# TUI-NICR/EMSANet

Hardware: AMD Instinct MI355X
Metric: images/sec (640x480 RGB-D, bs=32/GPU) fwd+bwd (higher is better)
Workload: dtype f32; 1 GPU; BASELINE.json configs[1]: full EMSANet RGB-D (resnet34-NBt1D x2, SE-add fusion, PPM, semantic+instance+orientation+scene heads), 640x480, bs=32/GPU, f32, train mode (BN batch stats, Dropout2d), step = fwd + bwd (fixed output cotangents) + grad all-reduce + SGD-nesterov update at lr 0 (fixed weights) replayed from a hipGraph; global_batch=32, parallelism=dp1, weights=random init (deterministic), mode=train-hipgraph

## Files before the change

emsanet_amd/_lib.py:

```python
import ctypes
import os
from ctypes import POINTER, Structure, c_char_p, c_float, c_int, c_int8, c_int32, c_int64, c_uint32, c_void_p

LIB_PATH = os.environ.get('EMSA_LIB') or os.path.join(
    os.path.dirname(os.path.abspath(__file__)), 'lib', 'libemsanet_hip.so')


class EmsaPackJob(Structure):
    _fields_ = [('src', c_void_p), ('dst0', c_void_p), ('dst1', c_void_p), ('cout', c_int32),
                ('cin', c_int32), ('kh', c_int32), ('kw', c_int32), ('kind', c_int32),
                ('first_block', c_int32), ('cout_total', c_int32), ('cout_off', c_int32),
                ('cin_total', c_int32), ('cin_off', c_int32)]


class EmsaDropoutJob(Structure):
    _fields_ = [('offset', c_int64), ('c', c_int32), ('layer_id', c_uint32), ('p', c_float),
                ('pad_', c_int32)]


class EmsaConvGeom(Structure):
    _fields_ = [
        ('n_img', c_int32),
        ('in_h', c_int32), ('in_w', c_int32),
        ('out_h', c_int32), ('out_w', c_int32),
# ... 27 lines not shown


_P = c_void_p
_GP = POINTER(EmsaConvGeom)
_TP = POINTER(EmsaTargetScale)

SIGNATURES = {
    'emsa_arch': (c_char_p, []),
    'emsa_version': (c_int, []),
    'emsa_set_batch_invariant': (c_int, [c_int]),
    'emsa_conv_igemm': (c_int, [_GP, _P, _P, _P, _P, _P, _P, _P, _P, c_int32, _P, c_int32, c_int32, _P]),
    'emsa_conv_stats_rows': (c_int, [_GP]),
    'emsa_conv1d_wino_supported': (c_int, [_GP]),
    'emsa_conv1d_wino_stats_rows': (c_int, [_GP]),
    'emsa_conv_relu_bits_words': (c_int64, [c_int64, c_int32]),
    'emsa_conv1d_wino_bnb': (c_int, [_GP, _P, _P, _P, _P, c_int32, _P, c_int32, _P, _P, _P, _P, _P,
                                     c_int32, _P]),
    'emsa_conv_igemm_bnb_t': (c_int, [c_int32, _GP, _P, _P, _P, _P, c_int32, _P, c_int32, _P, _P, _P, _P,
                                      _P, c_int32, _P]),
    'emsa_bn_bwd_apply_rows_t': (c_int, [c_int32, _P, _P, _P, _P, _P, _P, c_int32, c_int32, c_int64,
                                         c_int32, c_int32, _P, _P, _P, _P]),
    'emsa_conv1d_wino': (c_int, [_GP, _P, _P, _P, _P, _P, _P, _P, _P, c_int32, _P, c_int32, c_int32, _P,
                                 _P, _P]),
    'emsa_memset_async': (c_int, [_P, c_int32, c_int64, _P]),
    'emsa_graph_count_nodes': (c_int, [_P, POINTER(c_int32), POINTER(c_int32), POINTER(c_int32)]),
    'emsa_graph_replace_memsets': (c_int, [_P, POINTER(c_int32)]),
    'emsa_dropout2d_mask_batch': (c_int, [_P, _P, c_int32, c_int32, c_int32, c_uint32, _P, _P]),
    'emsa_to_nhwc_t': (c_int, [c_int32, _P, _P, c_int32, c_int32, c_int32, c_int32, c_int64, c_int64,
                               c_int64, c_int64, _P]),
    'emsa_conv1d_wino_resmask_supported': (c_int, [_GP, c_int32]),
    'emsa_conv1d_wino_resmask': (c_int, [_GP, _P, _P, _P, _P, c_int32, _P, _P]),
    'emsa_bn_act_fwd_wbits': (c_int, [_P, _P, _P, _P, _P, _P, c_int32, c_int64, c_int32, c_int32, _P, _P]),
    'emsa_bn_act_fwd_raff': (c_int, [_P] * 8 + [c_int32, c_int64, c_int32, c_int32, _P, c_int32, _P]),
    'emsa_bn_bwd_reduce_wbits': (c_int, [_P, _P, _P, _P, _P, _P, c_int32, c_int64, c_int32, _P, _P]),
    'emsa_bn_bwd_apply_wbits': (c_int, [_P] * 8 + [c_int32, c_int32, c_int64, c_int32, c_int32] + [_P] * 5),
    'emsa_conv1d_wino_inbn': (c_int, [_GP, _P, _P, _P, _P, _P, _P, _P, c_int32, _P, _P]),
    'emsa_conv_wgrad_inbn': (c_int, [_GP, _P, _P, _P, _P, _P, _P, _P, _P]),
    'emsa_conv_wgrad_inbn_t': (c_int, [c_int32, _GP, _P, _P, _P, _P, _P, _P, _P, _P]),
    'emsa_conv_wgrad_multi_inbn_t': (c_int, [c_int32, c_int32, _GP, POINTER(c_void_p), POINTER(c_void_p),
                                             POINTER(c_void_p), POINTER(c_void_p), _P,
                                             POINTER(c_void_p), POINTER(c_void_p), _P]),
    'emsa_conv1d_rs_inbn_t': (c_int, [c_int32, _GP, _P, _P, _P, _P, _P, _P, _P, c_int32, _P]),
    'emsa_bn_bwd_reduce_aff_t': (c_int, [c_int32, _P, _P, _P, _P, _P, _P, c_int32, c_int64, c_int32, _P, _P]),
    'emsa_bn_bwd_apply_aff_t': (c_int, [c_int32, _P, _P, _P, _P, _P, _P, _P, _P, c_int32, c_int32, c_int64,
                                        c_int32, _P, _P, _P, _P]),
    'emsa_conv_wgrad_multi_ws_bytes': (c_int64, [c_int32, c_int32, _GP]),
    'emsa_conv_wgrad_multi_t': (c_int, [c_int32, c_int32, _GP, POINTER(c_void_p), POINTER(c_void_p),
                                        POINTER(c_void_p), POINTER(c_void_p), _P, _P]),
    'emsa_pack_wino': (c_int, [_P, _P, _P, c_int32, c_int32, c_int32, _P]),
    'emsa_pack_batch': (c_int, [_P, c_int32, c_int32, _P]),
    'emsa_conv_wino2d_supported': (c_int, [_GP]),
    'emsa_conv_wino2d_stats_rows': (c_int, [_GP]),
    'emsa_conv_wino2d': (c_int, [_GP, _P, _P, _P, _P, _P, _P, _P, _P, c_int32, _P, c_int32, c_int32, _P]),
    'emsa_conv_wgrad_wino2d_supported': (c_int, [c_int32, _GP]),
    'emsa_conv_wgrad_wino2d_ws_bytes': (c_int64, [c_int32, _GP]),
    'emsa_conv_wgrad_wino2d_split_steps': (c_int, [c_int32, _GP]),
    'emsa_conv_wgrad_wino2d': (c_int, [c_int32, _GP, _P, _P, _P, _P, _P, c_int32, _P]),
    'emsa_pack_wino2d': (c_int, [_P, _P, _P, c_int32, c_int32, _P]),
    'emsa_pack_wino2d_packed': (c_int, [_P, _P, c_int32, c_int32, c_int32, _P]),
    'emsa_pack_wino_packed': (c_int, [_P, _P, c_int32, c_int32, c_int32, c_int32, _P]),
    'emsa_conv_wgrad_ws_bytes': (c_int64, [_GP]),
    'emsa_conv_wgrad': (c_int, [_GP, _P, _P, _P, _P, _P, _P]),
    'emsa_pack_weight_fwd': (c_int, [_P, _P] + [c_int32] * 8 + [_P]),
    'emsa_pack_weight_dgrad': (c_int, [_P, _P] + [c_int32] * 8 + [_P]),
    'emsa_unpack_wgrad': (c_int, [_P, _P] + [c_int32] * 8 + [_P]),
    'emsa_pack_weight_pair': (c_int, [_P, _P, _P] + [c_int32] * 4 + [_P]),
    'emsa_stem_pack_input': (c_int, [_P, _P, c_int32, c_int32, c_int32, c_int32, _P]),
    'emsa_stem_pack_weight': (c_int, [_P, _P, c_int32, c_int32, _P]),
    'emsa_stem_pack_input_rows_t': (c_int, [c_int32, _P, _P, c_int32, c_int32, c_int32, _P]),
    'emsa_stem_pack_weight_rows_t': (c_int, [c_int32, _P, _P, c_int32, _P]),
    'emsa_stem_unpack_wgrad_rows': (c_int, [_P, _P, c_int32, _P]),
    'emsa_stem_unpack_wgrad': (c_int, [_P, _P, c_int32, c_int32, _P]),
    'emsa_bn_finalize': (c_int, [_P, c_int32, c_int32, c_int64, _P, _P, c_float, c_float,
                                 _P, _P, _P, _P, _P, _P, _P, _P]),
    'emsa_bn_finalize_ws_bytes': (c_int, [c_int32]),
    'emsa_bn_fold': (c_int, [_P, _P, _P, _P, c_float, c_int32, _P, _P, _P, _P]),
    'emsa_relu_mask_words': (c_int64, [c_int64]),
    'emsa_bn_act_fwd': (c_int, [_P, _P, _P, _P, _P, _P, c_int32, c_int64, c_int32, c_int32, _P,
                                _P]),
    'emsa_bn_bwd_reduce': (c_int, [_P, _P, _P, _P, _P, _P, _P, c_int32, c_int64, c_int32, c_int32,
                                   _P, _P]),
    'emsa_bn_bwd_rows': (c_int, [c_int64, c_int32]),
    'emsa_bn_bwd_apply': (c_int, [_P, _P, _P, _P, _P, _P, _P, _P, _P, c_int32, c_int32, c_int64,
                                  c_int32, c_int32, c_int32, _P, _P, _P, _P, _P]),
    'emsa_dropout2d_mask': (c_int, [_P, c_int32, c_int32, c_float, c_uint32, c_uint32, _P]),
    'emsa_maxpool3x3s2_fwd': (c_int, [_P, _P, _P, c_int32, c_int32, c_int32, c_int32, _P]),
    'emsa_maxpool3x3s2_bwd': (c_int, [_P, _P, _P, c_int32, c_int32, c_int32, c_int32, _P]),
    'emsa_channel_ws_floats': (c_int, [c_int32, c_int64, c_int32]),
    'emsa_channel_mean': (c_int, [_P, _P, _P, c_int32, c_int64, c_int32, _P]),
    'emsa_se_mlp_fwd': (c_int, [_P] * 7 + [c_int32] * 3 + [_P]),
    'emsa_se_mlp_bwd': (c_int, [_P] * 11 + [c_int32] * 3 + [_P]),
    'emsa_se_scale_add_fwd': (c_int, [_P] * 5 + [c_int32, c_int64, c_int32, _P]),
    'emsa_se_scale_bwd_reduce': (c_int, [_P, _P, _P, _P, c_int32, c_int64, c_int32, _P]),
    'emsa_se_scale_bwd_apply': (c_int, [_P] * 5 + [c_int32, c_int64, c_int32, _P]),
    'emsa_up2x_dw3x3_fwd': (c_int, [_P] * 5 + [c_int32] * 4 + [_P]),
    'emsa_up2x_dw3x3_fwd_skipbn': (c_int, [_P] * 7 + [c_int32] * 4 + [_P]),
    'emsa_up2x_dw3x3_bwd_data': (c_int, [_P] * 3 + [c_int32] * 4 + [_P]),
    'emsa_up2x_dw3x3_bwd_weight': (c_int, [_P] * 4 + [c_int32] * 4 + [_P]),
    'emsa_up2x_dw3x3_bwd': (c_int, [_P] * 6 + [c_int32] * 4 + [_P]),
    'emsa_up2x_dw3x3_bwd_supported': (c_int, [c_int32, c_int32]),
    'emsa_adaptive_avgpool_fwd': (c_int, [_P, _P] + [c_int32] * 5 + [_P]),
    'emsa_adaptive_avgpool_bwd': (c_int, [_P, _P] + [c_int32] * 6 + [_P]),
    'emsa_bilinear_fwd': (c_int, [_P, _P] + [c_int32] * 7 + [_P]),
    'emsa_bilinear_bwd': (c_int, [_P, _P] + [c_int32] * 7 + [_P]),
    'emsa_head_act_fwd': (c_int, [_P, _P, c_int64] + [c_int32] * 5 + [_P]),
    'emsa_head_act_bwd': (c_int, [_P, _P, _P, _P, c_int64] + [c_int32] * 5 + [_P]),
# ... 185 lines not shown
```

emsanet_amd/csrc/conv_wino.hip:

```cpp
#include <cstdlib>

#include "common.h"
#include "prof.h"

namespace {

constexpr int kWK = 16;
constexpr int kWLD = kWK;
constexpr int kPairs = 32;

typedef unsigned int u32x4w __attribute__((ext_vector_type(4)));
typedef __bf16 wbf16x8 __attribute__((ext_vector_type(8)));
constexpr uint32_t kOOBw = 0x80000000u;
__device__ __forceinline__ __amdgpu_buffer_rsrc_t wrsrc(const void* p, uint32_t bytes) {
  return __builtin_amdgcn_make_buffer_rsrc(const_cast<void*>(p), 0, (int)bytes, 0x00020000);
}
__device__ __forceinline__ float4 wbuf_ld4(__amdgpu_buffer_rsrc_t r, uint32_t off) {
  return __builtin_bit_cast(float4, __builtin_amdgcn_raw_buffer_load_b128(r, (int)off, 0, 0));
}
__device__ __forceinline__ float4 wbuf_ld4s(__amdgpu_buffer_rsrc_t r, uint32_t voff, uint32_t soff) {
  return __builtin_bit_cast(float4,
                            __builtin_amdgcn_raw_buffer_load_b128(r, (int)voff, (int)soff, 0));
}
typedef float wf32x2 __attribute__((ext_vector_type(2)));
// ... 214 lines not shown
        acc[u] = __builtin_amdgcn_mfma_f32_32x32x2f32(v.z, fb[u].z, acc[u], 0, 0, 0);
#pragma unroll
      for (int u = 0; u < NT; ++u)
        acc[u] = __builtin_amdgcn_mfma_f32_32x32x2f32(v.w, fb[u].w, acc[u], 0, 0, 0);
    }
    }
#if EMSA_WINO_PRIO != 0
    __builtin_amdgcn_s_setprio(0);
#endif
    __syncthreads();
    if (has_next) store_lds(s + 1);
    __syncthreads();
  }

  constexpr int SLD = kWN + 4;
  constexpr int HP = kPairs / 2;
  constexpr uint32_t kNoPix = 0xFFFFFFFFu;
  float* const stage = smem;
  const int col4 = tid % NC4, n = n0 + col4 * 4;
  const int rgi = tid / NC4;
  const bool nok = n < p.n_ch;
  uint32_t lane_pix = kNoPix;
  {
    const int q = q0 + (lane >> 1);
    if (q < p.MP) {
      const int line = (int)wdiv((uint32_t)q, p.mul_pl, p.sh_pl);
      const int pp = q - line * p.PL;
      const int img = (int)wdiv((uint32_t)line, p.mul_a, p.sh_a);
      const int a = line - img * p.A;
      const int b = 2 * pp + (lane & 1);
      if (b < p.L) lane_pix = (uint32_t)(img * p.px_simg + a * p.px_sa + b * p.px_sb);
    }
  }
  wf32x2 ylo[PXI], yhi[PXI];
  uint32_t opix[PXI];
  bool ok[PXI];
  const float4 bv = (nok && p.bias) ? emsa_ld4(p.bias + n) : emsa_zero4();
  const wf32x2 blo = {bv.x, bv.y}, bhi = {bv.z, bv.w};
  const float sgo = (rgi & 1) ? -1.f : 1.f;
  const wf32x2 sg2o = {sgo, sgo};
  const int m03row = (rgi & 1) ? 3 : 0;
#pragma unroll
  for (int k = 0; k < PXI; ++k) {
    const uint32_t o = (uint32_t)__builtin_amdgcn_ds_bpermute((rgi + RG * k) * 4, (int)lane_pix);
    ok[k] = nok && o != kNoPix;
    opix[k] = o;
  }
  const __amdgpu_buffer_rsrc_t rs_out = wrsrc(p.out, kOOBw);
  const __amdgpu_buffer_rsrc_t rs_res = wrsrc(p.residual, kOOBw);
  const __amdgpu_buffer_rsrc_t rs_msk = wrsrc(p.mask_src, kOOBw);
  const __amdgpu_buffer_rsrc_t rs_mb = wrsrc(p.mask_bits, kOOBw);
  float4 rres[PXI], rmsk[PXI];
  wu32x2 rbits[PXI];
#pragma unroll
  for (int k = 0; k < PXI; ++k) {
    const bool live = ok[k];
    if (p.residual)
      rres[k] = wbuf_ld4(rs_res, live ? (opix[k] * (uint32_t)p.ld_res + (uint32_t)n) * 4u : kOOBw);
    if (p.mask_src)
      rmsk[k] = wbuf_ld4(rs_msk, live ? (opix[k] * (uint32_t)p.ld_mask + (uint32_t)n) * 4u : kOOBw);
    if constexpr (kWN == 64) {
      if (p.mask_bits)
        rbits[k] = __builtin_bit_cast(
            wu32x2, __builtin_amdgcn_raw_buffer_load_b64(
                        rs_mb, (int)(live ? (opix[k] * (uint32_t)p.tiles_n + (uint32_t)nt) * 8u
                                          : kOOBw), 0, 0));
    }
  }
#pragma unroll
  for (int h = 0; h < 2; ++h) {
  if (h) __syncthreads();
#pragma unroll
  for (int t = 0; t < NT; ++t)
#pragma unroll
    for (int r = 8 * h; r < 8 * h + 8; ++r) {
      const int row = (r & 3) + 8 * (r >> 2) + 4 * lh;
      stage[(wave * HP + row - HP * h) * SLD + t * 32 + l31] = acc[t][r];
    }
  __syncthreads();
#pragma unroll
  for (int k = h * (PXI / 2); k < (h + 1) * (PXI / 2); ++k) {
    const int px = rgi + RG * k;
    const int prl = (px >> 1) - HP * h;
    const float4 m1 = emsa_ld4(stage + (1 * HP + prl) * SLD + col4 * 4);
    const float4 m2 = emsa_ld4(stage + (2 * HP + prl) * SLD + col4 * 4);
    const float4 m03 = emsa_ld4(stage + (m03row * HP + prl) * SLD + col4 * 4);
    const wf32x2 tlo = wf32x2{m2.x, m2.y} + wf32x2{m03.x, m03.y};
    const wf32x2 thi = wf32x2{m2.z, m2.w} + wf32x2{m03.z, m03.w};
    ylo[k] = __builtin_elementwise_fma(tlo, sg2o, wf32x2{m1.x, m1.y}) + blo;
    yhi[k] = __builtin_elementwise_fma(thi, sg2o, wf32x2{m1.z, m1.w}) + bhi;
  }
  }

  if (p.stats != nullptr) {
    __syncthreads();
    float* red = smem;
    float* tmean = smem + RG * kWN;
    int* scnt = reinterpret_cast<int*>(tmean + kWN);
    wf32x2 s1lo = {0.f, 0.f}, s1hi = {0.f, 0.f};
    float wgt[PXI];
    int cnt = 0;
#pragma unroll
    for (int k = 0; k < PXI; ++k) {
      wgt[k] = ok[k] ? 1.f : 0.f;
      const wf32x2 w2 = {wgt[k], wgt[k]};
      s1lo = __builtin_elementwise_fma(ylo[k], w2, s1lo);
      s1hi = __builtin_elementwise_fma(yhi[k], w2, s1hi);
      cnt += ok[k] ? 1 : 0;
    }
    emsa_st4(red + rgi * kWN + col4 * 4, make_float4(s1lo.x, s1lo.y, s1hi.x, s1hi.y));
    if (col4 == 0) scnt[rgi] = cnt;
    __syncthreads();
    if (tid < kWN) {
      float a1 = 0.f;
#pragma unroll
      for (int g = 0; g < RG; ++g) a1 += red[g * kWN + tid];
      int c = 0;
#pragma unroll
      for (int g = 0; g < RG; ++g) c += scnt[g];
// ... 528 lines not shown
```

emsanet_amd/csrc/conv_wino2d.hip:

```cpp
#include "common.h"
#include "prof.h"

namespace {

constexpr int kK2 = 8;
constexpr int kTiles = 32;

typedef unsigned int u32x4v __attribute__((ext_vector_type(4)));
typedef float vf32x2 __attribute__((ext_vector_type(2)));
constexpr uint32_t kOOBw = 0x80000000u;
__device__ __forceinline__ __amdgpu_buffer_rsrc_t vrsrc(const void* p, uint32_t bytes) {
  return __builtin_amdgcn_make_buffer_rsrc(const_cast<void*>(p), 0, (int)bytes, 0x00020000);
}
__device__ __forceinline__ float4 vbuf_ld4(__amdgpu_buffer_rsrc_t r, uint32_t off) {
  return __builtin_bit_cast(float4, __builtin_amdgcn_raw_buffer_load_b128(r, (int)off, 0, 0));
}
__device__ __forceinline__ float4 vbuf_ld4s(__amdgpu_buffer_rsrc_t r, uint32_t voff, uint32_t soff) {
  return __builtin_bit_cast(float4,
                            __builtin_amdgcn_raw_buffer_load_b128(r, (int)voff, (int)soff, 0));
}
__device__ __forceinline__ uint32_t vdiv(uint32_t n, uint32_t mul, uint32_t sh) {
  return (__umulhi(n, mul) + n) >> sh;
}
__device__ __forceinline__ float4 sub4(float4 a, float4 b) {
  const vf32x2 lo = vf32x2{a.x, a.y} - vf32x2{b.x, b.y}, hi = vf32x2{a.z, a.w} - vf32x2{b.z, b.w};
  return make_float4(lo.x, lo.y, hi.x, hi.y);
}
__device__ __forceinline__ float4 add4(float4 a, float4 b) {
  const vf32x2 lo = vf32x2{a.x, a.y} + vf32x2{b.x, b.y}, hi = vf32x2{a.z, a.w} + vf32x2{b.z, b.w};
  return make_float4(lo.x, lo.y, hi.x, hi.y);
}

struct Wino2dArgs {
  const float* in;
  const float* u;
  float* out;
  const float* bias;
  float* stats;
  const float* scale;
  const float* shift;
  const float* residual;
  const float* mask_src;
  int ld_out, ld_res, ld_mask, act;
  int H, W, TH, TW, MT;
  int k_ch, n_ch;
  int in_simg, in_srow, in_spx;
  int tiles_m, tiles_n, ksteps;
  uint32_t in_bytes, u_bytes;
  uint32_t mul_tw, sh_tw, mul_th, sh_th;
};

template <int NT>
__global__ __launch_bounds__(256, NT == 1 ? 4 : 2) void conv_wino2d_kernel(const Wino2dArgs p) {
  constexpr int WN = 32 * NT;
  constexpr int NC4 = WN / 4;
  constexpr int RG = 256 / NC4;
  constexpr int PXH = 64 / RG;
  constexpr int PXI = 2 * PXH;
  constexpr int BLD = 16 * WN * 2 / 256;
  extern __shared__ __attribute__((aligned(16))) float smem[];
  float* const Hs = smem;
  float* const Us = smem + 16 * kTiles * kK2;

  const int tid = threadIdx.x, lane = tid & 63, wave = __builtin_amdgcn_readfirstlane(tid >> 6);
  const int l31 = lane & 31, lh = lane >> 5;
  const int wg = emsa_xcd_remap(blockIdx.x, gridDim.x);
  const int nt = wg % p.tiles_n, mt = wg / p.tiles_n;
  const int q0 = mt * kTiles, n0 = nt * WN;
  const __amdgpu_buffer_rsrc_t rs_in = vrsrc(p.in, p.in_bytes);
  const __amdgpu_buffer_rsrc_t rs_u = vrsrc(p.u, p.u_bytes);

  const int c4 = (tid & 1) * 4;
  const int ltile = (tid >> 1) & 31;
  uint32_t a_voff[4], b_voff[BLD];
  {
    const int q = q0 + ltile;
    int base = 0, y0 = 0;
    bool xok = false;
    if (q < p.MT) {
      const int line = (int)vdiv((uint32_t)q, p.mul_tw, p.sh_tw);
      const int tx = q - line * p.TW;
      const int img = (int)vdiv((uint32_t)line, p.mul_th, p.sh_th);
      const int ty = line - img * p.TH;
      const int x = 2 * tx - 1 + wave;
      y0 = 2 * ty;
      xok = x >= 0 && x < p.W;
      base = img * p.in_simg + y0 * p.in_srow + x * p.in_spx + c4;
    }
#pragma unroll
    for (int r = 0; r < 4; ++r) {
      const int y = y0 + r - 1;
      const bool ok = xok && y >= 0 && y < p.H;
      a_voff[r] = ok ? (uint32_t)(base + (r - 1) * p.in_srow) * 4u : kOOBw;
    }
  }
#pragma unroll
  for (int j = 0; j < BLD; ++j) {
    const int f = (tid >> 1) + 128 * j;
    const int comp = f / WN, n = n0 + (f % WN);
    b_voff[j] = n < p.n_ch ? (uint32_t)((comp * p.ksteps * p.n_ch + n) * kK2 + c4) * 4u : kOOBw;
  }
  const uint32_t last_oob = (p.ksteps - 1) * kK2 + c4 < p.k_ch ? 0u : kOOBw;
  float4 ra[4], rb[BLD];
  auto load_regs = [&](int s) {
    const uint32_t so = (uint32_t)(s * kK2) * 4u, sou = (uint32_t)(s * p.n_ch * kK2) * 4u;
    const uint32_t pm = (s + 1) * kK2 > p.k_ch ? 0xFFFFFFFFu : 0u;
#pragma unroll
    for (int r = 0; r < 4; ++r) ra[r] = vbuf_ld4s(rs_in, a_voff[r] | (last_oob & pm), so);
#pragma unroll
    for (int j = 0; j < BLD; ++j) rb[j] = vbuf_ld4s(rs_u, b_voff[j] | (last_oob & pm), sou);
  };
  auto store_lds = [&]() {
    float* const h = Hs + (wave * kTiles + ltile) * kK2 + c4;
    emsa_st4(h + 0 * 4 * kTiles * kK2, sub4(ra[0], ra[2]));
    emsa_st4(h + 1 * 4 * kTiles * kK2, add4(ra[1], ra[2]));
    emsa_st4(h + 2 * 4 * kTiles * kK2, sub4(ra[2], ra[1]));
    emsa_st4(h + 3 * 4 * kTiles * kK2, sub4(ra[1], ra[3]));
#pragma unroll
    for (int j = 0; j < BLD; ++j) emsa_st4(Us + ((tid >> 1) + 128 * j) * kK2 + c4, rb[j]);
  };

  const int ca = wave == 0 ? 0 : wave == 2 ? 2 : 1;
  const int cb = wave == 2 ? 1 : wave == 3 ? 3 : 2;
  const float sg = wave == 1 ? 1.f : -1.f;

  load_regs(0);
  f32x16 acc[4][NT];
#pragma unroll
  for (int i = 0; i < 4; ++i)
#pragma unroll
    for (int t = 0; t < NT; ++t)
#pragma unroll
      for (int r = 0; r < 16; ++r) acc[i][t][r] = 0.f;
  store_lds();
  __syncthreads();
  const float* const a0 = Hs + (ca * kTiles + l31) * kK2 + lh * 4;
  const float* const a1 = Hs + (cb * kTiles + l31) * kK2 + lh * 4;
  const float* const b = Us + (wave * WN + l31) * kK2 + lh * 4;
  for (int s = 0; s < p.ksteps; ++s) {
    const bool has_next = s + 1 < p.ksteps;
    __builtin_amdgcn_s_setprio(3);
    if (has_next) load_regs(s + 1);
    __builtin_amdgcn_s_setprio(1);
#pragma unroll
    for (int i = 0; i < 4; ++i) {
      const float4 x0 = emsa_ld4(a0 + i * 4 * kTiles * kK2), x1 = emsa_ld4(a1 + i * 4 * kTiles * kK2);
      const vf32x2 sg2 = {sg, sg};
      const vf32x2 vlo = __builtin_elementwise_fma(vf32x2{x1.x, x1.y}, sg2, vf32x2{x0.x, x0.y});
      const vf32x2 vhi = __builtin_elementwise_fma(vf32x2{x1.z, x1.w}, sg2, vf32x2{x0.z, x0.w});
      float4 fb[NT];
#pragma unroll
      for (int u = 0; u < NT; ++u) fb[u] = emsa_ld4(b + (i * 4 * WN + u * 32) * kK2);
#pragma unroll
      for (int u = 0; u < NT; ++u)
        acc[i][u] = __builtin_amdgcn_mfma_f32_32x32x2f32(vlo.x, fb[u].x, acc[i][u], 0, 0, 0);
#pragma unroll
      for (int u = 0; u < NT; ++u)
        acc[i][u] = __builtin_amdgcn_mfma_f32_32x32x2f32(vlo.y, fb[u].y, acc[i][u], 0, 0, 0);
#pragma unroll
      for (int u = 0; u < NT; ++u)
        acc[i][u] = __builtin_amdgcn_mfma_f32_32x32x2f32(vhi.x, fb[u].z, acc[i][u], 0, 0, 0);
#pragma unroll
      for (int u = 0; u < NT; ++u)
        acc[i][u] = __builtin_amdgcn_mfma_f32_32x32x2f32(vhi.y, fb[u].w, acc[i][u], 0, 0, 0);
    }
    __builtin_amdgcn_s_setprio(0);
    __syncthreads();
    if (has_next) store_lds();
    __syncthreads();
  }

  constexpr int SLD = WN + 4;
  constexpr uint32_t kNoPix = 0xFFFFFFFFu;
  float* const stage = smem;
  const int col4 = tid % NC4, n = n0 + col4 * 4;
  const int rgi = tid / NC4;
  const bool nok = n < p.n_ch;
  uint32_t lane_pix[2] = {kNoPix, kNoPix};
  {
    const int q = q0 + (lane >> 1);
    if (q < p.MT) {
      const int line = (int)vdiv((uint32_t)q, p.mul_tw, p.sh_tw);
      const int tx = q - line * p.TW;
      const int img = (int)vdiv((uint32_t)line, p.mul_th, p.sh_th);
      const int ty = line - img * p.TH;
      const int x = 2 * tx + (lane & 1);
#pragma unroll
      for (int a = 0; a < 2; ++a) {
        const int y = 2 * ty + a;
        if (x < p.W && y < p.H) lane_pix[a] = (uint32_t)((img * p.H + y) * p.W + x);
      }
    }
  }
  vf32x2 ylo[PXI], yhi[PXI];
  uint32_t opix[PXI];
  bool ok[PXI];
  const float4 bv = (nok && p.bias) ? emsa_ld4(p.bias + n) : emsa_zero4();
  const vf32x2 blo = {bv.x, bv.y}, bhi = {bv.z, bv.w};
  const float sgo = (rgi & 1) ? -1.f : 1.f;
  const vf32x2 sg2o = {sgo, sgo};
  const int m03row = (rgi & 1) ? 3 : 0;
#pragma unroll
  for (int k = 0; k < PXI; ++k) {
    const int a = k / PXH, kk = k % PXH;
    const uint32_t o = (uint32_t)__builtin_amdgcn_ds_bpermute((rgi + RG * kk) * 4, (int)lane_pix[a]);
    ok[k] = nok && o != kNoPix;
    opix[k] = o;
  }
  const __amdgpu_buffer_rsrc_t rs_out = vrsrc(p.out, kOOBw);
  const __amdgpu_buffer_rsrc_t rs_res = vrsrc(p.residual, kOOBw);
  const __amdgpu_buffer_rsrc_t rs_msk = vrsrc(p.mask_src, kOOBw);
  float4 rres[PXI], rmsk[PXI];
#pragma unroll
  for (int k = 0; k < PXI; ++k) {
    const bool live = ok[k];
    if (p.residual)
      rres[k] = vbuf_ld4(rs_res, live ? (opix[k] * (uint32_t)p.ld_res + (uint32_t)n) * 4u : kOOBw);
    if (p.mask_src)
      rmsk[k] = vbuf_ld4(rs_msk, live ? (opix[k] * (uint32_t)p.ld_mask + (uint32_t)n) * 4u : kOOBw);
  }
#pragma unroll
  for (int a = 0; a < 2; ++a) {
    __syncthreads();
#pragma unroll
    for (int t = 0; t < NT; ++t)
#pragma unroll
      for (int r = 0; r < 16; ++r) {
        const int row = (r & 3) + 8 * (r >> 2) + 4 * lh;
        const float v = a == 0 ? (acc[0][t][r] + acc[1][t][r]) + acc[2][t][r]
                               : (acc[1][t][r] - acc[2][t][r]) - acc[3][t][r];
        stage[(wave * kTiles + row) * SLD + t * 32 + l31] = v;
      }
    __syncthreads();
#pragma unroll
    for (int kk = 0; kk < PXH; ++kk) {
      const int k = a * PXH + kk;
      const int tl = (rgi + RG * kk) >> 1;
      const float4 m1 = emsa_ld4(stage + (1 * kTiles + tl) * SLD + col4 * 4);
      const float4 m2 = emsa_ld4(stage + (2 * kTiles + tl) * SLD + col4 * 4);
      const float4 m03 = emsa_ld4(stage + (m03row * kTiles + tl) * SLD + col4 * 4);
      const vf32x2 tlo = vf32x2{m2.x, m2.y} + vf32x2{m03.x, m03.y};
      const vf32x2 thi = vf32x2{m2.z, m2.w} + vf32x2{m03.z, m03.w};
      ylo[k] = __builtin_elementwise_fma(tlo, sg2o, vf32x2{m1.x, m1.y}) + blo;
      yhi[k] = __builtin_elementwise_fma(thi, sg2o, vf32x2{m1.z, m1.w}) + bhi;
    }
  }

  if (p.stats != nullptr) {
    __syncthreads();
    float* red = smem;
    float* tmean = smem + RG * WN;
    int* scnt = reinterpret_cast<int*>(tmean + WN);
    vf32x2 s1lo = {0.f, 0.f}, s1hi = {0.f, 0.f};
    float wgt[PXI];
    int cnt = 0;
#pragma unroll
    for (int k = 0; k < PXI; ++k) {
      wgt[k] = ok[k] ? 1.f : 0.f;
      const vf32x2 w2 = {wgt[k], wgt[k]};
      s1lo = __builtin_elementwise_fma(ylo[k], w2, s1lo);
      s1hi = __builtin_elementwise_fma(yhi[k], w2, s1hi);
      cnt += ok[k] ? 1 : 0;
    }
    emsa_st4(red + rgi * WN + col4 * 4, make_float4(s1lo.x, s1lo.y, s1hi.x, s1hi.y));
    if (col4 == 0) scnt[rgi] = cnt;
    __syncthreads();
    if (tid < WN) {
      float a1 = 0.f;
#pragma unroll
      for (int g = 0; g < RG; ++g) a1 += red[g * WN + tid];
      int c = 0;
#pragma unroll
// ... 50 lines not shown
      if (p.mask_src) {
        const float4 mm = rmsk[k];
        v.x = mm.x > 0.f ? v.x : 0.f; v.y = mm.y > 0.f ? v.y : 0.f;
        v.z = mm.z > 0.f ? v.z : 0.f; v.w = mm.w > 0.f ? v.w : 0.f;
      }
      if (p.act == EMSA_ACT_RELU) {
        v.x = fmaxf(v.x, 0.f); v.y = fmaxf(v.y, 0.f);
        v.z = fmaxf(v.z, 0.f); v.w = fmaxf(v.w, 0.f);
      }
      const uint32_t off = live ? (opix[k] * (uint32_t)p.ld_out + (uint32_t)n) * 4u : kOOBw;
      __builtin_amdgcn_raw_buffer_store_b128(__builtin_bit_cast(u32x4v, v), rs_out, (int)off, 0, 0);
    }
  }
}

__global__ void pack_wino2d_kernel(const float* __restrict__ w, float* __restrict__ u,
                                   float* __restrict__ ud, int cout, int cin) {
  const int total = cout * cin;
  for (int i = blockIdx.x * blockDim.x + threadIdx.x; i < total; i += gridDim.x * blockDim.x) {
    const int ci = i % cin, co = i / cin;
    float g[9], v[16];
#pragma unroll
    for (int t = 0; t < 9; ++t) g[t] = w[(size_t)i * 9 + t];
    emsa_wino2d_u(g, v);
#pragma unroll
    for (int c = 0; c < 16; ++c) {
      if (u) u[emsa_wino2d_at(c, co, ci, cout, cin)] = v[c];
      if (ud) ud[emsa_wino2d_at(emsa_wino2d_flip(c), ci, co, cin, cout)] = v[c];
    }
  }
}

__global__ void pack_wino2d_packed_kernel(const float* __restrict__ wp, float* __restrict__ u,
                                          int n, int k, int flip) {
  const int total = n * k;
  const size_t NK = (size_t)total;
  for (int i = blockIdx.x * blockDim.x + threadIdx.x; i < total; i += gridDim.x * blockDim.x) {
    float g[9], v[16];
#pragma unroll
    for (int t = 0; t < 9; ++t) g[t] = wp[(size_t)(flip ? 8 - t : t) * NK + i];
    emsa_wino2d_u(g, v);
#pragma unroll
    for (int c = 0; c < 16; ++c) u[emsa_wino2d_at(c, i / k, i % k, n, k)] = v[c];
  }
}

inline void magic2(uint32_t d, uint32_t& mul, uint32_t& sh) {
  uint32_t s = 0;
  while ((1ull << s) < d) ++s;
  sh = s;
  mul = (uint32_t)(((1ull << 32) * ((1ull << s) - d)) / d + 1);
}

}

extern "C" int emsa_pack_wino2d(const float* w_oihw, float* u, float* u_dgrad, int32_t cout,
                                int32_t cin, void* stream) {
  if (!w_oihw || (!u && !u_dgrad)) return EMSA_E_ARG;
  if (cout < 1 || cin < 1) return EMSA_E_SHAPE;
  int grid = (cout * cin + 255) / 256;
  if (grid > 2048) grid = 2048;
  hipLaunchKernelGGL(pack_wino2d_kernel, dim3(grid), dim3(256), 0, (hipStream_t)stream, w_oihw, u,
                     u_dgrad, cout, cin);
  return emsa_launch_status();
}

extern "C" int emsa_pack_wino2d_packed(const float* w_packed, float* u, int32_t n_ch, int32_t k_ch,
                                       int32_t flip, void* stream) {
  if (!w_packed || !u) return EMSA_E_ARG;
  if (n_ch < 1 || k_ch < 1) return EMSA_E_SHAPE;
  int grid = (n_ch * k_ch + 255) / 256;
  if (grid > 2048) grid = 2048;
  hipLaunchKernelGGL(pack_wino2d_packed_kernel, dim3(grid), dim3(256), 0, (hipStream_t)stream,
                     w_packed, u, n_ch, k_ch, flip ? 1 : 0);
  return emsa_launch_status();
}

extern "C" int emsa_conv_wino2d_supported(const EmsaConvGeom* g) {
  if (!g) return 0;
  if (g->out_pix_img || g->out_pix_row || g->out_pix_px || g->out_pix_off) return 0;
  auto tap3 = [](int off, int step) { return (off == -1 || off == 1) && step == -off; };
  if (!(g->kh == 3 && g->kw == 3 && tap3(g->off_w, g->step_w) && tap3(g->off_h, g->step_h) &&
        g->off_h == g->off_w))
    return 0;
  if (g->mul_h != 1 || g->mul_w != 1 || g->div_h != 1 || g->div_w != 1) return 0;
  if (g->n_img < 1 || g->in_h < 1 || g->in_w < 1 || g->k_ch < 4 || g->n_ch < 4) return 0;
  if (g->in_h != g->out_h || g->in_w != g->out_w) return 0;
  if ((g->k_ch & 3) || (g->n_ch & 3) || (g->ld_out & 3) || (g->in_px_stride & 3) ||
      (g->in_row_stride & 3) || (g->in_img_stride & 3))
    return 0;
  if ((long)g->n_img * g->in_img_stride >= (1L << 29)) return 0;
  if ((long)16 * g->n_ch * (g->k_ch + 7) >= (1L << 29)) return 0;
  return 1;
}

extern "C" int emsa_conv_wino2d_stats_rows(const EmsaConvGeom* g) {
  if (!emsa_conv_wino2d_supported(g)) return EMSA_E_SHAPE;
  const long mtl = (long)g->n_img * ((g->out_h + 1) / 2) * ((g->out_w + 1) / 2);
  return (int)((mtl + kTiles - 1) / kTiles);
}

extern "C" int emsa_conv_wino2d(const EmsaConvGeom* g, const float* in, const float* u2, float* out,
                                const float* bias, float* stats, const float* scale,
                                const float* shift, const float* residual, int32_t ld_res,
                                const float* mask_src, int32_t ld_mask, int32_t act,
                                void* stream) {
  if (!emsa_conv_wino2d_supported(g)) return EMSA_E_SHAPE;
  if (!in || !u2 || !out) return EMSA_E_ARG;
  if ((scale == nullptr) != (shift == nullptr)) return EMSA_E_ARG;
  if (stats && (scale || residual || mask_src || act != EMSA_ACT_NONE)) return EMSA_E_SHAPE;
  if (act != EMSA_ACT_NONE && act != EMSA_ACT_RELU) return EMSA_E_SHAPE;
  auto al16 = [](const void* q) { return (((uintptr_t)q) & 15) == 0; };
  if (!al16(in) || !al16(u2) || !al16(out) || !al16(bias) || !al16(scale) || !al16(shift) ||
      (residual && (!al16(residual) || (ld_res & 3))) ||
      (mask_src && (!al16(mask_src) || (ld_mask & 3))))
    return EMSA_E_SHAPE;
  Wino2dArgs a;
  a.in = in; a.u = u2; a.out = out; a.bias = bias; a.stats = stats; a.scale = scale;
  a.shift = shift; a.residual = residual; a.mask_src = mask_src;
  a.ld_out = g->ld_out; a.ld_res = ld_res; a.ld_mask = ld_mask; a.act = act;
  a.H = g->out_h; a.W = g->out_w;
  a.TH = (a.H + 1) / 2; a.TW = (a.W + 1) / 2;
  const long mtl = (long)g->n_img * a.TH * a.TW;
  {
    const long px = (long)g->n_img * a.H * a.W, lim = 1L << 29;
    if (px * g->ld_out >= lim || (residual && px * ld_res >= lim) ||
        (mask_src && px * ld_mask >= lim))
      return EMSA_E_SHAPE;
  }
  a.MT = (int)mtl;
  a.k_ch = g->k_ch; a.n_ch = g->n_ch;
  a.in_simg = (int)g->in_img_stride; a.in_srow = (int)g->in_row_stride; a.in_spx = g->in_px_stride;
  const int nt = g->n_ch % 64 == 0 ? 2 : 1;
  const int wn = 32 * nt;
  a.tiles_m = (a.MT + kTiles - 1) / kTiles;
  a.tiles_n = (g->n_ch + wn - 1) / wn;
  a.ksteps = (g->k_ch + kK2 - 1) / kK2;
  a.in_bytes = (uint32_t)((size_t)g->n_img * g->in_img_stride * sizeof(float));
  a.u_bytes = (uint32_t)((size_t)16 * a.ksteps * kK2 * g->n_ch * sizeof(float));
  magic2((uint32_t)a.TW, a.mul_tw, a.sh_tw);
  magic2((uint32_t)a.TH, a.mul_th, a.sh_th);
  const size_t lds_main = (size_t)(16 * kTiles + 16 * wn) * kK2 * sizeof(float);
  const size_t lds_epi = (size_t)4 * kTiles * (wn + 4) * sizeof(float);
  const size_t lds = lds_main > lds_epi ? lds_main : lds_epi;
  const double flops = 2.0 * g->n_img * a.H * a.W * (double)g->k_ch * g->n_ch * 9.0;
  const int ps = emsa_prof_begin(kProfClassWino3x3, flops, (hipStream_t)stream);
  if (nt == 2)
    hipLaunchKernelGGL((conv_wino2d_kernel<2>), dim3(a.tiles_m * a.tiles_n), dim3(256), lds,
                       (hipStream_t)stream, a);
  else
    hipLaunchKernelGGL((conv_wino2d_kernel<1>), dim3(a.tiles_m * a.tiles_n), dim3(256), lds,
                       (hipStream_t)stream, a);
  emsa_prof_end(ps, (hipStream_t)stream);
  return emsa_launch_status();
}
```

include/emsanet_hip.h:

```cpp
#ifndef EMSANET_HIP_H
#define EMSANET_HIP_H

#include <stdint.h>

#ifdef __cplusplus
extern "C" {
#endif

#define EMSA_OK 0
#define EMSA_E_SHAPE (-1)
#define EMSA_E_ARG (-2)
#define EMSA_E_LAUNCH (-3)

#define EMSA_ACT_NONE 0
#define EMSA_ACT_RELU 1

#define EMSA_DT_F32 0
#define EMSA_DT_BF16 1
#define EMSA_DT_F16 2

const char* emsa_arch(void);
int emsa_version(void);
int emsa_set_batch_invariant(int on);

// ... 4 lines not shown
  int32_t k_ch;
  int32_t n_ch;
  int32_t kh, kw;
  int32_t mul_h, off_h, step_h, div_h;
  int32_t mul_w, off_w, step_w, div_w;
  int64_t in_img_stride, in_row_stride;
  int32_t in_px_stride;
  int32_t ld_out;
  int32_t out_pix_img, out_pix_row, out_pix_px, out_pix_off;
} EmsaConvGeom;

int emsa_conv_igemm(const EmsaConvGeom* g, const float* in, const float* w, float* out,
                    const float* bias, float* stats, const float* scale, const float* shift,
                    const float* residual, int32_t ld_res, const float* mask_src,
                    int32_t ld_mask, int32_t act, void* stream);
int emsa_conv_stats_rows(const EmsaConvGeom* g);

int64_t emsa_conv_wgrad_ws_bytes(const EmsaConvGeom* g);
int emsa_conv_wgrad(const EmsaConvGeom* g, const float* in, const float* dout, float* dw,
                    float* dbias, float* ws, void* stream);

int emsa_conv1d_wino_supported(const EmsaConvGeom* g);
int emsa_conv1d_wino_stats_rows(const EmsaConvGeom* g);
int64_t emsa_conv_relu_bits_words(int64_t pixels, int32_t n_ch);
int emsa_conv1d_wino(const EmsaConvGeom* g, const float* in, const float* u, float* out,
                     const float* bias, float* stats, const float* scale, const float* shift,
                     const float* residual, int32_t ld_res, const float* mask_src,
                     int32_t ld_mask, int32_t act, const uint64_t* mask_bits,
                     uint64_t* relu_bits, void* stream);
int emsa_conv1d_wino_bnb(const EmsaConvGeom* g, const float* dy, const float* u, float* out,
                         const float* residual, int32_t ld_res, const float* t, int32_t ld_t,
                         const float* bn_scale, const float* bn_shift, const float* bn_mean,
                         const float* bn_invstd, float* partial, int32_t rows_alloc, void* stream);
int emsa_conv1d_wino_resmask_supported(const EmsaConvGeom* g, int32_t ld_res);
int emsa_conv1d_wino_resmask(const EmsaConvGeom* g, const float* dy, const float* u, float* out,
                             const float* residual, int32_t ld_res, const uint64_t* res_bits,
                             void* stream);
int emsa_conv1d_wino_inbn(const EmsaConvGeom* g, const float* in, const float* u, float* out,
                          const float* bias, float* stats, const float* in_scale,
                          const float* in_shift, int32_t act, uint64_t* relu_bits, void* stream);
int emsa_conv_wgrad_inbn(const EmsaConvGeom* g, const float* in, const float* dout, float* dw,
                         float* dbias, float* ws, const float* in_scale, const float* in_shift,
                         void* stream);
int emsa_pack_wino(const float* w_oihw, float* u, float* u_dgrad, int32_t cout, int32_t cin,
                   int32_t rows, void* stream);
int emsa_pack_wino_packed(const float* w_packed, float* u, int32_t n_ch, int32_t k_ch,
                          int32_t rows, int32_t flip, void* stream);
int emsa_conv_wino2d_supported(const EmsaConvGeom* g);
int emsa_conv_wino2d_stats_rows(const EmsaConvGeom* g);
int emsa_conv_wino2d(const EmsaConvGeom* g, const float* in, const float* u2, float* out,
                     const float* bias, float* stats, const float* scale, const float* shift,
                     const float* residual, int32_t ld_res, const float* mask_src,
                     int32_t ld_mask, int32_t act, void* stream);
int emsa_conv_wgrad_wino2d_supported(int32_t dtype, const EmsaConvGeom* g);
int64_t emsa_conv_wgrad_wino2d_ws_bytes(int32_t dtype, const EmsaConvGeom* g);
int emsa_conv_wgrad_wino2d_split_steps(int32_t dtype, const EmsaConvGeom* g);
int emsa_conv_wgrad_wino2d(int32_t dtype, const EmsaConvGeom* g, const void* in, const void* dout,
                           float* dw, float* dbias, float* ws, int32_t packed, void* stream);
int emsa_pack_wino2d(const float* w_oihw, float* u, float* u_dgrad, int32_t cout, int32_t cin,
                     void* stream);
int emsa_pack_wino2d_packed(const float* w_packed, float* u, int32_t n_ch, int32_t k_ch,
                            int32_t flip, void* stream);
typedef struct EmsaPackJob {
  const float* src;
  float* dst0;
  float* dst1;
  int32_t cout, cin, kh, kw;
  int32_t kind;
  int32_t first_block;
  int32_t cout_total, cout_off, cin_total, cin_off;
} EmsaPackJob;
int emsa_pack_batch(const EmsaPackJob* jobs_device, int32_t n_jobs, int32_t total_blocks,
                    void* stream);

int emsa_pack_weight_fwd(const float* w_oihw, float* w_packed, int32_t cout, int32_t cin,
                         int32_t kh, int32_t kw, int32_t cout_total, int32_t cout_off,
                         int32_t cin_total, int32_t cin_off,
                         void* stream);
int emsa_pack_weight_dgrad(const float* w_oihw, float* w_packed, int32_t cout, int32_t cin,
                           int32_t kh, int32_t kw, int32_t cout_total, int32_t cout_off,
                           int32_t cin_total, int32_t cin_off,
                           void* stream);
int emsa_pack_weight_pair(const float* w_oihw, float* w_packed_fwd, float* w_packed_dgrad,
                          int32_t cout, int32_t cin, int32_t kh, int32_t kw, void* stream);
int emsa_unpack_wgrad(const float* dw_packed, float* dw_oihw, int32_t cout, int32_t cin,
                      int32_t kh, int32_t kw, int32_t cout_total, int32_t cout_off,
                      int32_t cin_total, int32_t cin_off,
                      void* stream);

int emsa_stem_pack_input(const float* x_nchw, float* x_pad, int32_t n, int32_t c, int32_t h,
                         int32_t w, void* stream);
int emsa_stem_pack_weight(const float* w_oihw, float* w_packed, int32_t cout, int32_t cin,
                          void* stream);
int emsa_stem_unpack_wgrad(const float* dw_packed, float* dw_oihw, int32_t cout, int32_t cin,
                           void* stream);
int emsa_stem_pack_input_rows_t(int32_t dtype, const float* x, void* xp, int32_t n, int32_t h,
                                int32_t w, void* stream);
int emsa_stem_pack_weight_rows_t(int32_t dtype, const float* w, void* wp, int32_t cout, void* stream);
int emsa_stem_unpack_wgrad_rows(const float* dwp, float* dw, int32_t cout, void* stream);

int emsa_bn_finalize(const float* stats, int32_t rows, int32_t c, int64_t count,
                     const float* gamma, const float* beta, float eps, float momentum,
                     float* running_mean, float* running_var, float* scale, float* shift,
                     float* save_mean, float* save_invstd, void* ws, void* stream);
int emsa_bn_finalize_ws_bytes(int32_t c);
int emsa_bn_fold(const float* gamma, const float* beta, const float* running_mean,
// ... 526 lines not shown
```

Baseline: 345.6 images/s.

## Stage two K steps of input per barrier in 2D Winograd conv kernel

Adds a KS=16 variant of the 2D Winograd forward kernel. It loads and transforms input tiles for two K steps at once, so input loads and stores happen every other step with wider per-thread loads. By default it is used when NT=2 and k_ch>=40, and it can be overridden through an env var or a setter. It also splits the epilogue residual and mask loads into per-flag loops. In exchange it doubles the input LDS buffer, which lowers occupancy bounds, and it adds ablation macros for experiments.

```diff
diff --git a/emsanet_amd/_lib.py b/emsanet_amd/_lib.py
--- a/emsanet_amd/_lib.py
+++ b/emsanet_amd/_lib.py
@@ -103,6 +103,7 @@
     'emsa_conv_wino2d_supported': (c_int, [_GP]),
     'emsa_conv_wino2d_stats_rows': (c_int, [_GP]),
     'emsa_conv_wino2d': (c_int, [_GP, _P, _P, _P, _P, _P, _P, _P, _P, c_int32, _P, c_int32, c_int32, _P]),
+    'emsa_wino2d_set_stage': (c_int, [c_int]),
     'emsa_conv_wgrad_wino2d_supported': (c_int, [c_int32, _GP]),
     'emsa_conv_wgrad_wino2d_ws_bytes': (c_int64, [c_int32, _GP]),
     'emsa_conv_wgrad_wino2d_split_steps': (c_int, [c_int32, _GP]),
diff --git a/emsanet_amd/csrc/conv_wino.hip b/emsanet_amd/csrc/conv_wino.hip
--- a/emsanet_amd/csrc/conv_wino.hip
+++ b/emsanet_amd/csrc/conv_wino.hip
@@ -290,19 +290,26 @@
   const __amdgpu_buffer_rsrc_t rs_mb = wrsrc(p.mask_bits, kOOBw);
   float4 rres[PXI], rmsk[PXI];
   wu32x2 rbits[PXI];
-#pragma unroll
-  for (int k = 0; k < PXI; ++k) {
-    const bool live = ok[k];
-    if (p.residual)
-      rres[k] = wbuf_ld4(rs_res, live ? (opix[k] * (uint32_t)p.ld_res + (uint32_t)n) * 4u : kOOBw);
-    if (p.mask_src)
-      rmsk[k] = wbuf_ld4(rs_msk, live ? (opix[k] * (uint32_t)p.ld_mask + (uint32_t)n) * 4u : kOOBw);
-    if constexpr (kWN == 64) {
-      if (p.mask_bits)
+  if (p.residual) {
+#pragma unroll
+    for (int k = 0; k < PXI; ++k)
+      rres[k] =
+          wbuf_ld4(rs_res, ok[k] ? (opix[k] * (uint32_t)p.ld_res + (uint32_t)n) * 4u : kOOBw);
+  }
+  if (p.mask_src) {
+#pragma unroll
+    for (int k = 0; k < PXI; ++k)
+      rmsk[k] =
+          wbuf_ld4(rs_msk, ok[k] ? (opix[k] * (uint32_t)p.ld_mask + (uint32_t)n) * 4u : kOOBw);
+  }
+  if constexpr (kWN == 64) {
+    if (p.mask_bits) {
+#pragma unroll
+      for (int k = 0; k < PXI; ++k)
         rbits[k] = __builtin_bit_cast(
             wu32x2, __builtin_amdgcn_raw_buffer_load_b64(
-                        rs_mb, (int)(live ? (opix[k] * (uint32_t)p.tiles_n + (uint32_t)nt) * 8u
-                                          : kOOBw), 0, 0));
+                        rs_mb, (int)(ok[k] ? (opix[k] * (uint32_t)p.tiles_n + (uint32_t)nt) * 8u
+                                           : kOOBw), 0, 0));
     }
   }
 #pragma unroll
diff --git a/emsanet_amd/csrc/conv_wino2d.hip b/emsanet_amd/csrc/conv_wino2d.hip
--- a/emsanet_amd/csrc/conv_wino2d.hip
+++ b/emsanet_amd/csrc/conv_wino2d.hip
@@ -50,9 +50,17 @@
   uint32_t mul_tw, sh_tw, mul_th, sh_th;
 };
 
-template <int NT>
-__global__ __launch_bounds__(256, NT == 1 ? 4 : 2) void conv_wino2d_kernel(const Wino2dArgs p) {
+#ifndef EMSA_W2D_ABL
+#define EMSA_W2D_ABL 0
+#endif
+
+template <int NT, int KS>
+__global__ __launch_bounds__(256, NT == 2 ? 2 : KS == 16 ? 3 : 4) void conv_wino2d_kernel(
+    const Wino2dArgs p) {
+  static_assert(KS == 8 || KS == 16, "input stage of one or two K steps");
   constexpr int WN = 32 * NT;
+  constexpr int HSZ = 16 * kTiles * kK2;
+  constexpr int NA = KS / 2;
   constexpr int NC4 = WN / 4;
   constexpr int RG = 256 / NC4;
   constexpr int PXH = 64 / RG;
@@ -60,7 +68,7 @@
   constexpr int BLD = 16 * WN * 2 / 256;
   extern __shared__ __attribute__((aligned(16))) float smem[];
   float* const Hs = smem;
-  float* const Us = smem + 16 * kTiles * kK2;
+  float* const Us = smem + (KS / kK2) * HSZ;
 
   const int tid = threadIdx.x, lane = tid & 63, wave = __builtin_amdgcn_readfirstlane(tid >> 6);
   const int l31 = lane & 31, lh = lane >> 5;
@@ -70,61 +78,104 @@
   const __amdgpu_buffer_rsrc_t rs_in = vrsrc(p.in, p.in_bytes);
   const __amdgpu_buffer_rsrc_t rs_u = vrsrc(p.u, p.u_bytes);
 
-  const int c4 = (tid & 1) * 4;
-  const int ltile = (tid >> 1) & 31;
-  uint32_t a_voff[4], b_voff[BLD];
+  const int c4 = KS == 8 ? (tid & 1) * 4 : (tid & 3) * 4;
+  const int ltile = KS == 8 ? (tid >> 1) & 31 : (tid >> 2) & 31;
+  const int col0 = KS == 8 ? wave : 2 * (wave >> 1);
+  const int cu4 = (tid & 1) * 4;
+  constexpr int NBV = KS == 16 ? 1 : BLD;
+  uint32_t a_voff[NA], b_voff[NBV];
   {
     const int q = q0 + ltile;
-    int base = 0, y0 = 0;
-    bool xok = false;
+    int base = 0, y0 = 0, x0 = 0;
+    bool qok = false;
     if (q < p.MT) {
       const int line = (int)vdiv((uint32_t)q, p.mul_tw, p.sh_tw);
       const int tx = q - line * p.TW;
       const int img = (int)vdiv((uint32_t)line, p.mul_th, p.sh_th);
       const int ty = line - img * p.TH;
-      const int x = 2 * tx - 1 + wave;
+      x0 = 2 * tx - 1 + col0;
       y0 = 2 * ty;
-      xok = x >= 0 && x < p.W;
-      base = img * p.in_simg + y0 * p.in_srow + x * p.in_spx + c4;
-    }
-#pragma unroll
-    for (int r = 0; r < 4; ++r) {
-      const int y = y0 + r - 1;
-      const bool ok = xok && y >= 0 && y < p.H;
-      a_voff[r] = ok ? (uint32_t)(base + (r - 1) * p.in_srow) * 4u : kOOBw;
-    }
-  }
-#pragma unroll
-  for (int j = 0; j < BLD; ++j) {
+      qok = true;
+      base = img * p.in_simg + y0 * p.in_srow + x0 * p.in_spx + c4;
+    }
+#pragma unroll
+    for (int cc = 0; cc < NA / 4; ++cc) {
+      const int x = x0 + cc;
+      const bool xok = qok && x >= 0 && x < p.W;
+#pragma unroll
+      for (int r = 0; r < 4; ++r) {
+        const int y = y0 + r - 1;
+        const bool ok = xok && y >= 0 && y < p.H;
+        a_voff[cc * 4 + r] =
+            ok ? (uint32_t)(base + cc * p.in_spx + (r - 1) * p.in_srow) * 4u : kOOBw;
+#if EMSA_W2D_ABL & 1
+        a_voff[cc * 4 + r] = kOOBw;
+#endif
+      }
+    }
+  }
+#pragma unroll
+  for (int j = 0; j < NBV; ++j) {
     const int f = (tid >> 1) + 128 * j;
     const int comp = f / WN, n = n0 + (f % WN);
-    b_voff[j] = n < p.n_ch ? (uint32_t)((comp * p.ksteps * p.n_ch + n) * kK2 + c4) * 4u : kOOBw;
-  }
-  const uint32_t last_oob = (p.ksteps - 1) * kK2 + c4 < p.k_ch ? 0u : kOOBw;
-  float4 ra[4], rb[BLD];
-  auto load_regs = [&](int s) {
-    const uint32_t so = (uint32_t)(s * kK2) * 4u, sou = (uint32_t)(s * p.n_ch * kK2) * 4u;
-    const uint32_t pm = (s + 1) * kK2 > p.k_ch ? 0xFFFFFFFFu : 0u;
-#pragma unroll
-    for (int r = 0; r < 4; ++r) ra[r] = vbuf_ld4s(rs_in, a_voff[r] | (last_oob & pm), so);
-#pragma unroll
-    for (int j = 0; j < BLD; ++j) rb[j] = vbuf_ld4s(rs_u, b_voff[j] | (last_oob & pm), sou);
+    b_voff[j] = n < p.n_ch ? (uint32_t)((comp * p.ksteps * p.n_ch + n) * kK2 + cu4) * 4u : kOOBw;
+#if EMSA_W2D_ABL & 2
+    b_voff[j] = kOOBw;
+#endif
+  }
+  const int stages = (p.k_ch + KS - 1) / KS;
+  const uint32_t last_oob_a = (stages - 1) * KS + c4 < p.k_ch ? 0u : kOOBw;
+  const uint32_t last_oob_b = (p.ksteps - 1) * kK2 + cu4 < p.k_ch ? 0u : kOOBw;
+  const uint32_t b_jstride = (uint32_t)((128 / WN) * p.ksteps * p.n_ch * kK2) * 4u;
+  float4 ra[NA], rb[BLD];
+  auto load_a = [&](int S) {
+    const uint32_t so = (uint32_t)(S * KS) * 4u;
+    if constexpr (KS == 16) {
+      const uint32_t oob = c4 < p.k_ch - S * KS ? 0u : kOOBw;
+#pragma unroll
+      for (int r = 0; r < NA; ++r) ra[r] = vbuf_ld4s(rs_in, a_voff[r] | oob, so);
+    } else {
+      const uint32_t pm = (S + 1) * KS > p.k_ch ? 0xFFFFFFFFu : 0u;
+#pragma unroll
+      for (int r = 0; r < NA; ++r) ra[r] = vbuf_ld4s(rs_in, a_voff[r] | (last_oob_a & pm), so);
+    }
   };
-  auto store_lds = [&]() {
-    float* const h = Hs + (wave * kTiles + ltile) * kK2 + c4;
-    emsa_st4(h + 0 * 4 * kTiles * kK2, sub4(ra[0], ra[2]));
-    emsa_st4(h + 1 * 4 * kTiles * kK2, add4(ra[1], ra[2]));
-    emsa_st4(h + 2 * 4 * kTiles * kK2, sub4(ra[2], ra[1]));
-    emsa_st4(h + 3 * 4 * kTiles * kK2, sub4(ra[1], ra[3]));
-#pragma unroll
-    for (int j = 0; j < BLD; ++j) emsa_st4(Us + ((tid >> 1) + 128 * j) * kK2 + c4, rb[j]);
+  auto load_b = [&](int s) {
+    const uint32_t sou = (uint32_t)(s * p.n_ch * kK2) * 4u;
+    if constexpr (KS == 16) {
+      const uint32_t voff = b_voff[0] | (cu4 < p.k_ch - s * kK2 ? 0u : kOOBw);
+#pragma unroll
+      for (int j = 0; j < BLD; ++j) rb[j] = vbuf_ld4s(rs_u, voff, sou + (uint32_t)j * b_jstride);
+    } else {
+      const uint32_t pm = (s + 1) * kK2 > p.k_ch ? 0xFFFFFFFFu : 0u;
+#pragma unroll
+      for (int j = 0; j < BLD; ++j) rb[j] = vbuf_ld4s(rs_u, b_voff[j] | (last_oob_b & pm), sou);
+    }
+  };
+  auto store_a = [&]() {
+    float* const h = Hs + (KS == 16 && (tid & 2) ? HSZ : 0) + (col0 * kTiles + ltile) * kK2 +
+                     (tid & 1) * 4;
+#pragma unroll
+    for (int cc = 0; cc < NA / 4; ++cc) {
+      const float4* const d = ra + cc * 4;
+      float* const hc = h + cc * kTiles * kK2;
+      emsa_st4(hc + 0 * 4 * kTiles * kK2, sub4(d[0], d[2]));
+      emsa_st4(hc + 1 * 4 * kTiles * kK2, add4(d[1], d[2]));
+      emsa_st4(hc + 2 * 4 * kTiles * kK2, sub4(d[2], d[1]));
+      emsa_st4(hc + 3 * 4 * kTiles * kK2, sub4(d[1], d[3]));
+    }
+  };
+  auto store_b = [&]() {
+#pragma unroll
+    for (int j = 0; j < BLD; ++j) emsa_st4(Us + ((tid >> 1) + 128 * j) * kK2 + cu4, rb[j]);
   };
 
   const int ca = wave == 0 ? 0 : wave == 2 ? 2 : 1;
   const int cb = wave == 2 ? 1 : wave == 3 ? 3 : 2;
   const float sg = wave == 1 ? 1.f : -1.f;
 
-  load_regs(0);
+  load_a(0);
+  load_b(0);
   f32x16 acc[4][NT];
 #pragma unroll
   for (int i = 0; i < 4; ++i)
@@ -132,19 +183,17 @@
     for (int t = 0; t < NT; ++t)
 #pragma unroll
       for (int r = 0; r < 16; ++r) acc[i][t][r] = 0.f;
-  store_lds();
+  store_a();
+  store_b();
   __syncthreads();
   const float* const a0 = Hs + (ca * kTiles + l31) * kK2 + lh * 4;
   const float* const a1 = Hs + (cb * kTiles + l31) * kK2 + lh * 4;
   const float* const b = Us + (wave * WN + l31) * kK2 + lh * 4;
-  for (int s = 0; s < p.ksteps; ++s) {
-    const bool has_next = s + 1 < p.ksteps;
-    __builtin_amdgcn_s_setprio(3);
-    if (has_next) load_regs(s + 1);
-    __builtin_amdgcn_s_setprio(1);
+  auto mma = [&](int half) {
 #pragma unroll
     for (int i = 0; i < 4; ++i) {
-      const float4 x0 = emsa_ld4(a0 + i * 4 * kTiles * kK2), x1 = emsa_ld4(a1 + i * 4 * kTiles * kK2);
+      const float4 x0 = emsa_ld4(a0 + half + i * 4 * kTiles * kK2),
+                   x1 = emsa_ld4(a1 + half + i * 4 * kTiles * kK2);
       const vf32x2 sg2 = {sg, sg};
       const vf32x2 vlo = __builtin_elementwise_fma(vf32x2{x1.x, x1.y}, sg2, vf32x2{x0.x, x0.y});
       const vf32x2 vhi = __builtin_elementwise_fma(vf32x2{x1.z, x1.w}, sg2, vf32x2{x0.z, x0.w});
@@ -164,10 +213,47 @@
       for (int u = 0; u < NT; ++u)
         acc[i][u] = __builtin_amdgcn_mfma_f32_32x32x2f32(vhi.y, fb[u].w, acc[i][u], 0, 0, 0);
     }
-    __builtin_amdgcn_s_setprio(0);
-    __syncthreads();
-    if (has_next) store_lds();
-    __syncthreads();
+  };
+  if constexpr (KS == 8) {
+    for (int s = 0; s < p.ksteps; ++s) {
+      const bool has_next = s + 1 < p.ksteps;
+      __builtin_amdgcn_s_setprio(3);
+      if (has_next) {
+        load_a(s + 1);
+        load_b(s + 1);
+      }
+      __builtin_amdgcn_s_setprio(1);
+      mma(0);
+      __builtin_amdgcn_s_setprio(0);
+      __syncthreads();
+      if (has_next) {
+        store_a();
+        store_b();
+      }
+      __syncthreads();
+    }
+  } else {
+    for (int S = 0; S < p.ksteps / 2; ++S) {
+      __builtin_amdgcn_s_setprio(3);
+      load_b(2 * S + 1);
+      load_a(S + 1);
+      __builtin_amdgcn_s_setprio(1);
+      mma(0);
+      __builtin_amdgcn_s_setprio(0);
+      __syncthreads();
+      store_b();
+      __syncthreads();
+      __builtin_amdgcn_s_setprio(3);
+      load_b(2 * S + 2);
+      __builtin_amdgcn_s_setprio(1);
+      mma(HSZ);
+      __builtin_amdgcn_s_setprio(0);
+      __syncthreads();
+      store_a();
+      store_b();
+      __syncthreads();
+    }
+    if (p.ksteps & 1) mma(0);
   }
 
   constexpr int SLD = WN + 4;
@@ -211,13 +297,17 @@
   const __amdgpu_buffer_rsrc_t rs_res = vrsrc(p.residual, kOOBw);
   const __amdgpu_buffer_rsrc_t rs_msk = vrsrc(p.mask_src, kOOBw);
   float4 rres[PXI], rmsk[PXI];
-#pragma unroll
-  for (int k = 0; k < PXI; ++k) {
-    const bool live = ok[k];
-    if (p.residual)
-      rres[k] = vbuf_ld4(rs_res, live ? (opix[k] * (uint32_t)p.ld_res + (uint32_t)n) * 4u : kOOBw);
-    if (p.mask_src)
-      rmsk[k] = vbuf_ld4(rs_msk, live ? (opix[k] * (uint32_t)p.ld_mask + (uint32_t)n) * 4u : kOOBw);
+  if (p.residual) {
+#pragma unroll
+    for (int k = 0; k < PXI; ++k)
+      rres[k] =
+          vbuf_ld4(rs_res, ok[k] ? (opix[k] * (uint32_t)p.ld_res + (uint32_t)n) * 4u : kOOBw);
+  }
+  if (p.mask_src) {
+#pragma unroll
+    for (int k = 0; k < PXI; ++k)
+      rmsk[k] =
+          vbuf_ld4(rs_msk, ok[k] ? (opix[k] * (uint32_t)p.ld_mask + (uint32_t)n) * 4u : kOOBw);
   }
 #pragma unroll
   for (int a = 0; a < 2; ++a) {
@@ -374,6 +464,24 @@
   mul = (uint32_t)(((1ull << 32) * ((1ull << s) - d)) / d + 1);
 }
 
+int g_wino2d_stage = [] {
+  const char* e = getenv("EMSA_WINO2D_STAGE");
+  const int v = e ? atoi(e) : 0;
+  return v == 8 || v == 16 ? v : 0;
+}();
+
+int wino2d_stage(int nt, int k_ch) {
+  if (k_ch <= kK2) return 8;
+  if (g_wino2d_stage) return g_wino2d_stage;
+  return nt == 2 && k_ch >= 40 ? 16 : 8;
+}
+
+}
+
+extern "C" int emsa_wino2d_set_stage(int ks) {
+  const int prev = g_wino2d_stage;
+  g_wino2d_stage = ks == 8 || ks == 16 ? ks : 0;
+  return prev;
 }
 
 extern "C" int emsa_pack_wino2d(const float* w_oihw, float* u, float* u_dgrad, int32_t cout,
@@ -462,17 +570,21 @@
   a.u_bytes = (uint32_t)((size_t)16 * a.ksteps * kK2 * g->n_ch * sizeof(float));
   magic2((uint32_t)a.TW, a.mul_tw, a.sh_tw);
   magic2((uint32_t)a.TH, a.mul_th, a.sh_th);
-  const size_t lds_main = (size_t)(16 * kTiles + 16 * wn) * kK2 * sizeof(float);
+  const int ks = wino2d_stage(nt, g->k_ch);
+  const size_t lds_main = (size_t)(16 * kTiles * (ks / kK2) + 16 * wn) * kK2 * sizeof(float);
   const size_t lds_epi = (size_t)4 * kTiles * (wn + 4) * sizeof(float);
   const size_t lds = lds_main > lds_epi ? lds_main : lds_epi;
   const double flops = 2.0 * g->n_img * a.H * a.W * (double)g->k_ch * g->n_ch * 9.0;
   const int ps = emsa_prof_begin(kProfClassWino3x3, flops, (hipStream_t)stream);
-  if (nt == 2)
-    hipLaunchKernelGGL((conv_wino2d_kernel<2>), dim3(a.tiles_m * a.tiles_n), dim3(256), lds,
-                       (hipStream_t)stream, a);
+  const dim3 grid(a.tiles_m * a.tiles_n), block(256);
+  if (nt == 2 && ks == 16)
+    hipLaunchKernelGGL((conv_wino2d_kernel<2, 16>), grid, block, lds, (hipStream_t)stream, a);
+  else if (nt == 2)
+    hipLaunchKernelGGL((conv_wino2d_kernel<2, 8>), grid, block, lds, (hipStream_t)stream, a);
+  else if (ks == 16)
+    hipLaunchKernelGGL((conv_wino2d_kernel<1, 16>), grid, block, lds, (hipStream_t)stream, a);
   else
-    hipLaunchKernelGGL((conv_wino2d_kernel<1>), dim3(a.tiles_m * a.tiles_n), dim3(256), lds,
-                       (hipStream_t)stream, a);
+    hipLaunchKernelGGL((conv_wino2d_kernel<1, 8>), grid, block, lds, (hipStream_t)stream, a);
   emsa_prof_end(ps, (hipStream_t)stream);
   return emsa_launch_status();
 }
diff --git a/include/emsanet_hip.h b/include/emsanet_hip.h
--- a/include/emsanet_hip.h
+++ b/include/emsanet_hip.h
@@ -80,6 +80,7 @@
                      const float* bias, float* stats, const float* scale, const float* shift,
                      const float* residual, int32_t ld_res, const float* mask_src,
                      int32_t ld_mask, int32_t act, void* stream);
+int emsa_wino2d_set_stage(int ks);
 int emsa_conv_wgrad_wino2d_supported(int32_t dtype, const EmsaConvGeom* g);
 int64_t emsa_conv_wgrad_wino2d_ws_bytes(int32_t dtype, const EmsaConvGeom* g);
 int emsa_conv_wgrad_wino2d_split_steps(int32_t dtype, const EmsaConvGeom* g);
```

After: 347.1 images/s (median of 6 runs). No clear change (+0.4%).
